# pyannote/pyannote-audio

Measured on AMD Instinct MI355X. Metric: audio-hours/sec (real-time factor) for speaker-diarization-3.1 pipeline, higher is better.
Workload: dtype f32

## Files before the change

include/pyannote_amd.h:

```cpp
#ifndef PYANNOTE_AMD_H
#define PYANNOTE_AMD_H

#include <stddef.h>
#include <stdint.h>

#ifdef __cplusplus
extern "C" {
#endif

int pa_version(void);
const char* pa_last_error(void);

void pa_prof_enable(int on);
size_t pa_prof_report(char* buf, size_t cap);

#define PA_MAX_LSTM_LAYERS 8
#define PA_MAX_LINEAR 4

typedef struct pa_seg_weights {
  int32_t sinc_stride;
  int32_t lstm_layers;
  int32_t lstm_hidden;
  int32_t lstm_bidir;
  int32_t num_linear;
// ... 42 lines not shown
int pa_sinc_fix_pool(const float* S, long Pc, int positions_per_chunk_step, int B, int P, const float* mean,
                     const float* rstd, float gamma, float beta, const float* filt_packed, float* tap_sums,
                     float* out, void* stream);
int pa_sinc_fir_span_centred(const float* wav, long wav_len, long span, const float* mean0, const float* rstd0,
                             const float* filt_packed, float* S, void* stream);
int pa_sinc_fix_pool_centred(const float* S, long Pc, int positions_per_chunk_step, int B, int P, const float* wav,
                             long wav_len, int N, const float* mean, const float* rstd, float gamma, float beta,
                             const float* filt_packed, float* tap_sums, float* out, void* stream);
int pa_conv5_pool(const float* xin, int B, int cin, int Lin, const float* in_mean,
                  const float* in_rstd, const float* gam, const float* bet, const float* w_packed,
                  const float* bias64, float* out, void* stream);
int pa_norm_transpose(const float* xin, int B, int T, const float* in_mean, const float* in_rstd,
                      const float* gam, const float* bet, float* X0, void* stream);
int pa_gemm_tn_ex(const float* A, int lda, const float* W, int ldw, const float* bias, const float* Res,
                  float* C, long ldc, int M, int N, int K, int act, int out_mode, void* stream);
int pa_gemm_tn(const float* A, int lda, const float* W, int ldw, const float* bias, float* C, long ldc,
               int M, int N, int K, int act, int out_mode, void* stream);
int pa_gemm_tn_s2(const float* X, int B, int H, int W, int cin, const float* Wt, int ldw, const float* bias, float* C,
                  long ldc, int N, void* stream);
int pa_lstm_rec(const float* xproj, const float* whh_packed, float* out, int ntiles, int ndir, int T,
                void* stream);
int pa_lstm_rec_h(const float* xproj, const float* whh_packed, float* out, int ntiles, int ndir, int T, int H,
                  void* stream);
int pa_classifier(const float* X, int ldx, int K, int ntiles, int T, int B, const float* cw,
                  const float* cb, int NC, const unsigned char* mapping, int S, float* logp,
                  unsigned char* multilabel, void* stream);

#define PA_MAX_RES_BLOCKS 128

typedef struct pa_emb_weights {
  int32_t num_mel;
  int32_t embed_dim;
  int32_t num_layers;
  int32_t num_blocks[4];
  int32_t planes[4];
  int32_t bottleneck;
  const float* fb_window;
  const float* fb_tw256;
  const float* fb_tw512;
  const float* fb_mel_w;
  const int32_t* fb_mel_lo;
  const int32_t* fb_mel_hi;
  const float* stem_w;
  const float* stem_shift;
  const float* blk_w1[PA_MAX_RES_BLOCKS];
  const float* blk_shift1[PA_MAX_RES_BLOCKS];
  const float* blk_w2[PA_MAX_RES_BLOCKS];
  const float* blk_shift2[PA_MAX_RES_BLOCKS];
  const float* blk_u1[PA_MAX_RES_BLOCKS];
  const float* blk_u2[PA_MAX_RES_BLOCKS];
  const float* blk_wsc[PA_MAX_RES_BLOCKS];
  const float* blk_shiftsc[PA_MAX_RES_BLOCKS];
  const float* blk_w3[PA_MAX_RES_BLOCKS];
  const float* blk_shift3[PA_MAX_RES_BLOCKS];
  const float* seg1_w;
  const float* seg1_b;
  const float* blk_v1[PA_MAX_RES_BLOCKS];
  const float* blk_v2[PA_MAX_RES_BLOCKS];
  int32_t fb_center_kernel;
} pa_emb_weights;

int pa_emb_num_fbank_frames(int num_samples);
int pa_emb_num_pool_frames(const pa_emb_weights* w, int num_samples);
size_t pa_emb_workspace_bytes(const pa_emb_weights* w, int num_chunks, int num_samples, int num_masks);
int pa_emb_forward(const pa_emb_weights* w, const float* wav, int64_t wav_len, int64_t chunk_stride,
                   int num_chunks, int num_samples, const float* masks, int num_masks, int mask_frames,
                   const int32_t* nearest_idx, float* emb, void* workspace, size_t workspace_bytes,
                   void* stream);

size_t pa_emb_ragged_workspace_bytes(const pa_emb_weights* w, int num_utterances, int max_samples);
int pa_emb_forward_ragged(const pa_emb_weights* w, const float* wav, int64_t wav_len, const int64_t* offsets,
                          const int32_t* lengths, int num_utterances, int max_samples, const float* masks, float* emb,
                          void* workspace, size_t workspace_bytes, void* stream);

size_t pa_emb_calibrate_workspace_bytes(const pa_emb_weights* w, int num_chunks, int num_samples);
int pa_emb_calibrate_winograd(const pa_emb_weights* w, const float* wav, int64_t wav_len, int64_t chunk_stride,
                              int num_chunks, int num_samples, float* report, float* emb, void* workspace,
                              size_t workspace_bytes, void* stream);
int pa_absmax_diff(const float* got, const float* ref, long n, float* out2, void* stream);

int pa_fbank(const float* wav, long wav_len, long chunk_stride, int B, int N, const float* window,
             const float* tw256, const float* tw512, const float* mel_w, const int* mel_lo,
             const int* mel_hi, int nmel, float* out, int center, void* stream);
int pa_fbank_center_span(const float* fb, int B, int T, int nmel, int kernel, float* out, void* stream);
int pa_resnet_stem(const float* fbank, int B, int T, int F, const float* w9, const float* shift,
                   float* out, void* stream);
int pa_conv3x3(const float* X, int B, int H, int W, int cin, const float* Wg, const float* shift,
               const float* R, float* Y, int cout, int stride, int relu, void* stream);
int pa_conv3x3_s2_sc_supported(int H, int cin, int cout);
int pa_conv3x3_s2_sc(const float* X, int B, int H, int W, int cin, const float* Wg, const float* shift,
                     const float* Wsc, const float* shift_sc, float* Y, float* Ysc, int cout, int relu,
                     void* stream);
int pa_winograd_pack_host(const float* conv_weight ,
                          const float* bn_scale , int cout, int cin,
                          float* U_slabs );
int pa_conv3x3_wino(const float* X, int B, int H, int W, int cin, const float* U, const float* shift,
                    const float* R, float* Y, int cout, int relu, void* stream);
int pa_winograd4_pack_host(const float* conv_weight ,
                           const float* bn_scale , int cout, int cin,
                           float* U_slabs );
int pa_conv3x3_wino4(const float* X, int B, int H, int W, int cin, const float* U, const float* shift,
                     const float* R, float* Y, int cout, int relu, void* stream);
int pa_conv3x3_wino4_rows(const float* X, int B, int H, int W, int cin, const float* U, const float* shift,
                          const float* R, float* Y, int cout, int relu, int rows, void* stream);
int pa_conv3x3_wino_rows(const float* X, int B, int H, int W, int cin, const float* U, const float* shift,
                         const float* R, float* Y, int cout, int relu, int y_first, void* stream);
int pa_stats_pool(const float* feat, int B, int Fh, int Tp, int C, const float* masks, int S, int Fm,
                  const int* nearest_idx, float* stats, void* stream);
int pa_fbank_ragged(const float* wav, long wav_len, const int64_t* offsets, const int32_t* lengths, int B,
                    int max_samples, const float* window, const float* tw256, const float* tw512, const float* mel_w,
                    const int* mel_lo, const int* mel_hi, int nmel, float* out, void* stream);
int pa_zero_tail_cols(float* x, int B, int H, int W, int C, const int32_t* lengths, int halvings, void* stream);
int pa_stats_pool_ragged(const float* feat, int B, int Fh, int W, int C, const int32_t* lengths, int halvings,
                         const float* masks, int ld_masks, float* stats, void* stream);

#define PA_W2V_MAX_CONV 8
#define PA_W2V_MAX_LAYERS 24
typedef struct pa_w2v_layer {
  const float* qk_w;
  const float* qk_b;
  const float* v_w;
  const float* out_w;
  const float* out_b;
  const float* ln1_g;
  const float* ln1_b;
  const float* ff1_w;
  const float* ff1_b;
  const float* ff2_w;
  const float* ff2_b;
  const float* ln2_g;
  const float* ln2_b;
  const float* gate_w;
  const float* gate_b;
  const float* gate_const;
} pa_w2v_layer;

typedef struct pa_sser_weights {
  int32_t num_conv;
  int32_t conv_channels[PA_W2V_MAX_CONV];
  int32_t conv_kernel[PA_W2V_MAX_CONV];
  int32_t conv_stride[PA_W2V_MAX_CONV];
  int32_t extractor_layer_norm;
  int32_t embed_dim, num_layers, num_heads, ff_dim, layer_norm_first;
  int32_t pos_kernel, pos_groups;
  int32_t wavlm;
  int32_t use_layer;
  int32_t lstm_layers, lstm_hidden, lstm_bidir, num_linear, linear_hidden, num_classes, num_speakers;
  const float* conv_w[PA_W2V_MAX_CONV];
  const float* conv_b[PA_W2V_MAX_CONV];
  const float* conv_norm_g[PA_W2V_MAX_CONV];
  const float* conv_norm_b[PA_W2V_MAX_CONV];
  const float* proj_ln_g;
  const float* proj_ln_b;
  const float* proj_w;
  const float* proj_b;
  const float* pos_w;
  const float* pos_b;
  const float* enc_ln_g;
  const float* enc_ln_b;
  pa_w2v_layer layers[PA_W2V_MAX_LAYERS];
  float layer_mix[PA_W2V_MAX_LAYERS];
  const float* lstm_wih[PA_MAX_LSTM_LAYERS];
  const float* lstm_bias[PA_MAX_LSTM_LAYERS];
  const float* lstm_whh[PA_MAX_LSTM_LAYERS];
  const float* lin_w[PA_MAX_LINEAR];
  const float* lin_b[PA_MAX_LINEAR];
// ... 249 lines not shown
```

pyannote-audio_amd/csrc/emb_fbank.hip:

```cpp
#include "common.h"

namespace pa {

constexpr int FB_WIN = 400, FB_SHIFT = 160, FB_NFFT = 512, FB_HALF = 256, FB_NBIN = 257;
constexpr int FB_FPB = 4;

struct cplx {
  float x, y;
};
__device__ __forceinline__ cplx cmul(cplx a, cplx b) {
  return {a.x * b.x - a.y * b.y, a.x * b.y + a.y * b.x};
}

template <bool kRagged>
__global__ __launch_bounds__(256) void k_fbank(const float* __restrict__ wav, long wav_len,
                                               long chunk_stride, int T, float scale, float preemph,
                                               const float* __restrict__ window,
                                               const float2* __restrict__ tw256,
                                               const float2* __restrict__ tw512,
                                               const float* __restrict__ mel_w,
                                               const int* __restrict__ mel_lo,
                                               const int* __restrict__ mel_hi, int nmel, float eps,
                                               float* __restrict__ out, const int64_t* __restrict__ offs,
                                               const int* __restrict__ lens) {
  __shared__ float2 bufA[FB_FPB][FB_HALF];
  __shared__ float2 bufB[FB_FPB][FB_HALF];
  __shared__ float2 s_tw256[FB_HALF];
  __shared__ float xs[FB_FPB][FB_NFFT + 1];
  const int tid = threadIdx.x, lane = tid & 63, wv = tid >> 6;
  const int b = blockIdx.y;
  const int t = blockIdx.x * FB_FPB + wv;
  int Tb = T;
  long base = (long)b * chunk_stride + (long)t * FB_SHIFT;
  if constexpr (kRagged) {
    const int n = lens[b];
    Tb = n < FB_WIN ? 0 : 1 + (n - FB_WIN) / FB_SHIFT;
    if ((int)blockIdx.x * FB_FPB >= Tb) return;
    base = offs[b] + (long)t * FB_SHIFT;
  }
  for (int i = tid; i < FB_HALF; i += 256) s_tw256[i] = tw256[i];
  const bool active = t < Tb;
  float2 w512[5];
#pragma unroll
  for (int i = 0; i < 5; ++i) w512[i] = lane + 64 * i <= FB_HALF ? tw512[lane + 64 * i] : make_float2(0.f, 0.f);

  float x[7];
  float s = 0.f;
#pragma unroll
  for (int i = 0; i < 7; ++i) {
    const int j = lane + 64 * i;
    float v = 0.f;
    if (active && j < FB_WIN) {
      const long g = base + j;
      v = (g < wav_len ? wav[g] : 0.f) * scale;
    }
    x[i] = v;
    s += v;
  }
  const float mean = wave_sum(s) / (float)FB_WIN;
  float* xw = xs[wv];
#pragma unroll
  for (int i = 0; i < 7; ++i) {
    const int j = lane + 64 * i;
    if (j < FB_WIN) xw[j + 1] = x[i] - mean;
  }
  if (lane == 0) xw[0] = x[0] - mean;
  __syncthreads();
  float y[8];
#pragma unroll
  for (int i = 0; i < 8; ++i) {
    const int j = lane + 64 * i;
    float v = 0.f;
    if (j < FB_WIN) v = (xw[j + 1] - preemph * xw[j]) * window[j];
    y[i] = v;
  }
  __syncthreads();
#pragma unroll
  for (int i = 0; i < 8; ++i) xw[lane + 64 * i] = y[i];
  __syncthreads();
  float2* A = bufA[wv];
  float2* Bf = bufB[wv];
#pragma unroll
  for (int i = 0; i < 4; ++i) {
    const int n = lane + 64 * i;
    A[n] = make_float2(xw[2 * n], xw[2 * n + 1]);
  }
  __syncthreads();

  float2* src = A;
  float2* dst = Bf;
#pragma unroll
  for (int pass = 0; pass < 4; ++pass) {
    const int Ns = 1 << (2 * pass);
    const int j = lane;
    const int k = j & (Ns - 1);
    const int tstep = 64 >> (2 * pass);
    cplx v[4];
#pragma unroll
    for (int r = 0; r < 4; ++r) {
      const float2 d = src[j + 64 * r];
      const float2 w = s_tw256[(r * k * tstep) & 255];
      v[r] = cmul({d.x, d.y}, {w.x, w.y});
    }
    const cplx t0 = {v[0].x + v[2].x, v[0].y + v[2].y};
    const cplx t1 = {v[0].x - v[2].x, v[0].y - v[2].y};
    const cplx t2 = {v[1].x + v[3].x, v[1].y + v[3].y};
    const cplx d13 = {v[1].x - v[3].x, v[1].y - v[3].y};
    const cplx t3 = {d13.y, -d13.x};
    const int j0 = ((j - k) << 2) + k;
    dst[j0] = make_float2(t0.x + t2.x, t0.y + t2.y);
    dst[j0 + Ns] = make_float2(t1.x + t3.x, t1.y + t3.y);
    dst[j0 + 2 * Ns] = make_float2(t0.x - t2.x, t0.y - t2.y);
    dst[j0 + 3 * Ns] = make_float2(t1.x - t3.x, t1.y - t3.y);
    __syncthreads();
    float2* tmp = src;
    src = dst;
    dst = tmp;
  }
#pragma unroll
  for (int i = 0; i < 5; ++i) {
    const int k = lane + 64 * i;
    if (k <= FB_HALF) {
      const float2 zk = src[k & 255];
      const float2 zc0 = src[(FB_HALF - k) & 255];
      const cplx zc = {zc0.x, -zc0.y};
      const cplx e = {0.5f * (zk.x + zc.x), 0.5f * (zk.y + zc.y)};
      const cplx dd = {0.5f * (zk.x - zc.x), 0.5f * (zk.y - zc.y)};
      const cplx o = {dd.y, -dd.x};
      const float2 w = w512[i];
      const cplx wo = cmul(o, {w.x, w.y});
      const float re = e.x + wo.x, im = e.y + wo.y;
      xw[k] = re * re + im * im;
    }
  }
  __syncthreads();
  if (active) {
    for (int m = lane; m < nmel; m += 64) {
      const float* wrow = mel_w + (long)m * FB_NBIN;
      float acc = 0.f;
      const int lo = mel_lo[m], hi = mel_hi[m];
      for (int k0 = lo; k0 <= hi; k0 += 8) {
        float wk[8];
#pragma unroll
        for (int u = 0; u < 8; ++u) wk[u] = k0 + u <= hi ? wrow[k0 + u] : 0.f;
#pragma unroll
        for (int u = 0; u < 8; ++u)
          if (k0 + u <= hi) acc = fmaf(xw[k0 + u], wk[u], acc);
      }
      out[((long)b * T + t) * nmel + m] = logf(fmaxf(acc, eps));
    }
  }
}

__global__ __launch_bounds__(320) void k_fbank_center(float* __restrict__ fb, int T, int nmel) {
  __shared__ float part[4][80];
  const int b = blockIdx.x;
  const int m = threadIdx.x % 80, p = threadIdx.x / 80;
  float* x = fb + (long)b * T * nmel;
  float s = 0.f;
  if (m < nmel)
    for (int t = p; t < T; t += 4) s += x[(long)t * nmel + m];
  part[p][m] = s;
  __syncthreads();
  const float mean = (part[0][m] + part[1][m] + part[2][m] + part[3][m]) / (float)T;
  if (m < nmel)
    for (int t = p; t < T; t += 4) x[(long)t * nmel + m] -= mean;
}

__global__ __launch_bounds__(320) void k_fbank_center_ragged(float* __restrict__ fb, int T, int nmel,
                                                             const int* __restrict__ lens) {
  __shared__ float part[4][80];
  const int b = blockIdx.x;
  const int m = threadIdx.x % 80, p = threadIdx.x / 80;
  const int n = lens[b];
  const int Tb = n < FB_WIN ? 0 : 1 + (n - FB_WIN) / FB_SHIFT;
  float* x = fb + (long)b * T * nmel;
  float s = 0.f;
  if (m < nmel)
    for (int t = p; t < Tb; t += 4) s += x[(long)t * nmel + m];
  part[p][m] = s;
  __syncthreads();
  const float mean = (part[0][m] + part[1][m] + part[2][m] + part[3][m]) / (float)Tb;
  if (m < nmel) {
    for (int t = p; t < Tb; t += 4) x[(long)t * nmel + m] -= mean;
    for (int t = Tb + p; t < T; t += 4) x[(long)t * nmel + m] = 0.f;
  }
}

constexpr int FC_TT = 240, FC_MG = 16, FC_KMAX = 2049;
__global__ __launch_bounds__(256) void k_fbank_center_span(const float* __restrict__ fb, int T, int nmel, int K,
                                                           float* __restrict__ out) {
  extern __shared__ float fc_tile[];
  const int b = blockIdx.z, m0 = blockIdx.y * FC_MG, t0 = blockIdx.x * FC_TT;
  const int half = K >> 1;
  const int m = threadIdx.x & (FC_MG - 1), tl = threadIdx.x >> 4;
  const float* x = fb + (long)b * T * nmel;
  const int rows = FC_TT + K - 1;
  for (int r = tl; r < rows; r += 16) {
    const int t = t0 - half + r;
    fc_tile[r * FC_MG + m] = (t >= 0 && t < T && m0 + m < nmel) ? x[(long)t * nmel + m0 + m] : 0.f;
  }
  __syncthreads();
  if (m0 + m >= nmel) return;
  for (int i = tl; i < FC_TT; i += 16) {
    const int t = t0 + i;
    if (t >= T) break;
    const int lo = t - half < 0 ? 0 : t - half, hi = t + half > T - 1 ? T - 1 : t + half;
    float s = 0.f;
    for (int u = lo; u <= hi; ++u) s += fc_tile[(u - t0 + half) * FC_MG + m];
    out[((long)b * T + t) * nmel + m0 + m] = fc_tile[(i + half) * FC_MG + m] - s / (float)(hi - lo + 1);
  }
}

}

extern "C" {

int pa_fbank_center_span(const float* fb, int B, int T, int nmel, int kernel, float* out, void* stream) {
  PA_REQUIRE(kernel >= 1 && (kernel & 1), "pa_fbank_center_span: the window must be an odd number of frames (got %d)",
             kernel);
  PA_REQUIRE(fb != out, "pa_fbank_center_span: works out of place");
  if (B <= 0 || T <= 0 || nmel <= 0) return 0;
  if (kernel > 2 * T - 1) kernel = 2 * T - 1;
  PA_REQUIRE(kernel <= pa::FC_KMAX,
             "pa_fbank_center_span: a running mean over %d frames of a %d-frame chunk needs more than the LDS holds "
             "(at most %d frames)", kernel, T, pa::FC_KMAX);
  const size_t lds = (size_t)(pa::FC_TT + kernel - 1) * pa::FC_MG * sizeof(float);
  static bool attr_set = false;
  if (!attr_set) {
    (void)hipFuncSetAttribute((const void*)pa::k_fbank_center_span, hipFuncAttributeMaxDynamicSharedMemorySize,
                              (int)((pa::FC_TT + pa::FC_KMAX - 1) * pa::FC_MG * sizeof(float)));
    attr_set = true;
  }
  hipLaunchKernelGGL(pa::k_fbank_center_span, dim3(pa::cdiv(T, pa::FC_TT), pa::cdiv(nmel, pa::FC_MG), B), dim3(256), lds,
                     (hipStream_t)stream, fb, T, nmel, kernel, out);
  PA_CHECK_LAUNCH("pa_fbank_center_span");
  return 0;
}

int pa_fbank(const float* wav, long wav_len, long chunk_stride, int B, int N, const float* window,
             const float* tw256, const float* tw512, const float* mel_w, const int* mel_lo,
             const int* mel_hi, int nmel, float* out, int center, void* stream) {
  PA_REQUIRE(nmel <= 80, "pa_fbank: at most 80 mel bins are built (got %d)", nmel);
  if (B <= 0) return 0;
  PA_REQUIRE(N >= pa::FB_WIN, "pa_fbank: %d samples is shorter than one 25 ms frame", N);
  const int T = 1 + (N - pa::FB_WIN) / pa::FB_SHIFT;
  hipStream_t st = (hipStream_t)stream;
  pa::ProfScope prof("k_fbank", stream, (double)B * T * (5.0 * 512 * 9 + 2.0 * 257 * 3 + 2.0 * 257 * 2),
                     4.0 * B * N + 4.0 * B * T * nmel * (center ? 3 : 1));
  hipLaunchKernelGGL(pa::k_fbank<false>, dim3(pa::cdiv(T, pa::FB_FPB), B), dim3(256), 0, st, wav, wav_len,
                     chunk_stride, T, 32768.0f, 0.97f, window, (const float2*)tw256,
                     (const float2*)tw512, mel_w, mel_lo, mel_hi, nmel, 1.1920928955078125e-07f, out,
                     (const int64_t*)nullptr, (const int*)nullptr);
  PA_CHECK_LAUNCH("pa_fbank");
  if (center) {
    hipLaunchKernelGGL(pa::k_fbank_center, dim3(B), dim3(320), 0, st, out, T, nmel);
    PA_CHECK_LAUNCH("pa_fbank_center");
  }
  return 0;
}

int pa_fbank_ragged(const float* wav, long wav_len, const int64_t* offsets, const int32_t* lengths, int B,
                    int max_samples, const float* window, const float* tw256, const float* tw512, const float* mel_w,
                    const int* mel_lo, const int* mel_hi, int nmel, float* out, void* stream) {
  PA_REQUIRE(nmel <= 80, "pa_fbank_ragged: at most 80 mel bins are built (got %d)", nmel);
  if (B <= 0) return 0;
  PA_REQUIRE(max_samples >= pa::FB_WIN, "pa_fbank_ragged: %d samples is shorter than one 25 ms frame", max_samples);
  const int T = 1 + (max_samples - pa::FB_WIN) / pa::FB_SHIFT;
  hipStream_t st = (hipStream_t)stream;
  pa::ProfScope prof("k_fbank_ragged", stream, (double)B * T * (5.0 * 512 * 9 + 2.0 * 257 * 3 + 2.0 * 257 * 2),
                     4.0 * B * max_samples + 12.0 * B * T * nmel);
  hipLaunchKernelGGL(pa::k_fbank<true>, dim3(pa::cdiv(T, pa::FB_FPB), B), dim3(256), 0, st, wav, wav_len, 0L, T,
                     32768.0f, 0.97f, window, (const float2*)tw256, (const float2*)tw512, mel_w, mel_lo, mel_hi, nmel,
                     1.1920928955078125e-07f, out, offsets, (const int*)lengths);
  PA_CHECK_LAUNCH("pa_fbank_ragged");
  hipLaunchKernelGGL(pa::k_fbank_center_ragged, dim3(B), dim3(320), 0, st, out, T, nmel, (const int*)lengths);
  PA_CHECK_LAUNCH("pa_fbank_center_ragged");
  return 0;
}

}
```

pyannote-audio_amd/csrc/emb_forward.cpp:

```cpp
#include "forward_common.h"

namespace {

struct EmbPlan {
  int B, N, T, F, S;
  int Hs[5], Ws[5];
  size_t fbank, act[4], stats, total, act_elems;
  size_t t2_off, gather_off;
};

inline bool s2_fold_wanted() {
  static const bool fold = getenv("PA_S2_FOLD") == nullptr || atoi(getenv("PA_S2_FOLD")) != 0;
  return fold;
}

inline bool prefer_wino4(int H, int W, int cin) {
  auto up = [](int a, int b) { return (long)((a + b - 1) / b) * b; };
  long p4 = up(H, 4) * up(W, 64);
  const long p4_lin = up(H, 4) * up(W, 4);
  if (p4_lin * 120 <= p4 * 100) p4 = p4_lin * 120 / 100;
  long p2 = up(H, 8) * up(W, 32);
  if (up(H, 4) * up(W, 64) < p2) p2 = up(H, 4) * up(W, 64);
  if (up(H, 2) * up(W, 128) < p2) p2 = up(H, 2) * up(W, 128);
  const long gain = cin >= 256 ? 130 : 122;
  return p4 * 100 <= p2 * gain;
}

bool make_plan(const pa_emb_weights* w, int B, int N, int S, EmbPlan* p, bool calib = false) {
  if (N < 400) return false;
  p->B = B;
  p->N = N;
  p->S = S < 1 ? 1 : S;
  p->T = 1 + (N - 400) / 160;
  p->F = w->num_mel;
  p->Hs[0] = p->F;
  p->Ws[0] = p->T;
  for (int l = 0; l < w->num_layers; ++l) {
    const int s = l == 0 ? 1 : 2;
    p->Hs[l + 1] = (p->Hs[l] - 1) / s + 1;
    p->Ws[l + 1] = (p->Ws[l] - 1) / s + 1;
  }
  pa::Bump ws;
  p->fbank = ws.take((size_t)B * p->T * p->F);
  const int ex = w->bottleneck ? 4 : 1;
  p->act_elems = (size_t)B * p->Hs[0] * p->Ws[0] * w->planes[0] * ex;
  for (int i = 0; i < 3; ++i) p->act[i] = ws.take(p->act_elems);
  p->t2_off = p->gather_off = 0;
  if (w->bottleneck) {
    size_t t1 = 0, t2 = 0, g = 0;
    int cin = w->planes[0];
    for (int l = 0; l < w->num_layers; ++l) {
      const size_t planes = w->planes[l];
      const size_t in_px = (size_t)B * p->Hs[l == 0 ? 1 : l] * p->Ws[l == 0 ? 1 : l];
      const size_t out_px = (size_t)B * p->Hs[l + 1] * p->Ws[l + 1];
      t1 = t1 > in_px * planes ? t1 : in_px * planes;
      t2 = t2 > out_px * planes ? t2 : out_px * planes;
      if (l > 0) g = g > out_px * cin ? g : out_px * cin;
      cin = 4 * (int)planes;
    }
    p->t2_off = pa::Bump::align(t1);
    p->gather_off = p->t2_off + pa::Bump::align(t2);
    p->act[3] = ws.take(p->gather_off + pa::Bump::align(g));
  } else if (calib) {
    p->act[3] = ws.take(p->act_elems);
  }
  const int L = w->num_layers;
  p->stats = ws.take((size_t)B * p->S * 2 * w->planes[L - 1] * ex * p->Hs[L]);
  p->total = ws.o;
  return true;
}

}

extern "C" {

int pa_emb_num_fbank_frames(int num_samples) {
  return num_samples < 400 ? 0 : 1 + (num_samples - 400) / 160;
}

int pa_emb_num_pool_frames(const pa_emb_weights* w, int num_samples) {
  EmbPlan p;
  if (!make_plan(w, 1, num_samples, 1, &p)) return 0;
  return p.Ws[w->num_layers];
}

size_t pa_emb_workspace_bytes(const pa_emb_weights* w, int num_chunks, int num_samples, int num_masks) {
  EmbPlan p;
  if (!make_plan(w, num_chunks, num_samples, num_masks, &p)) return 0;
  return p.total * sizeof(float);
}

}


static int emb_forward_impl(const pa_emb_weights* w, const float* wav, int64_t wav_len, int64_t chunk_stride,
                            int num_chunks, int num_samples, const float* masks, int num_masks, int mask_frames,
                            const int32_t* nearest_idx, float* emb, void* workspace, size_t workspace_bytes,
                            void* stream, float* calib, const int64_t* offsets = nullptr,
                            const int32_t* lengths = nullptr) {
  if (num_chunks <= 0) return 0;
  const bool ragged = lengths != nullptr;
  EmbPlan p;
  if (w->num_layers != 4 || !make_plan(w, num_chunks, num_samples, masks ? num_masks : 1, &p, calib != nullptr)) {
    pa::set_error("pa_emb_forward: %d samples is too short (fbank needs >= 400) or bad layer count",
                  num_samples);
    return 3;
  }
  if (workspace_bytes < p.total * sizeof(float)) {
    pa::set_error("pa_emb_forward: workspace too small (%zu < %zu bytes)", workspace_bytes,
                  p.total * sizeof(float));
    return 3;
  }
  float* ws = (float*)workspace;
  const int B = p.B;

  const int span = w->fb_center_kernel;
  if (ragged && span != 0) {
    pa::set_error("pa_emb_forward_ragged: fbank_centering_span checkpoints run one launch sequence per length");
    return 3;
  }
  if (ragged)
    PA_RUN(pa_fbank_ragged(wav, wav_len, offsets, lengths, B, p.N, w->fb_window, w->fb_tw256, w->fb_tw512, w->fb_mel_w,
                           w->fb_mel_lo, w->fb_mel_hi, w->num_mel, ws + p.fbank, stream));
  else
    PA_RUN(pa_fbank(wav, wav_len, chunk_stride, B, p.N, w->fb_window, w->fb_tw256, w->fb_tw512, w->fb_mel_w,
                    w->fb_mel_lo, w->fb_mel_hi, w->num_mel, ws + p.fbank, span == 0 ? 1 : 0, stream));
  auto zero_tail = [&](float* X, int l, int C) -> int {
    return ragged ? pa_zero_tail_cols(X, B, p.Hs[l], p.Ws[l], C, lengths, l > 0 ? l - 1 : 0, stream) : 0;
  };
  float* cur = ws + p.act[0];
  float* f1 = ws + p.act[1];
  float* f2 = ws + p.act[2];
  const float* feats = ws + p.fbank;
  if (span != 0) {
    PA_RUN(pa_fbank_center_span(ws + p.fbank, B, p.T, p.F, span, f1, stream));
    feats = f1;
  }
  PA_RUN(pa_resnet_stem(feats, B, p.T, p.F, w->stem_w, w->stem_shift, cur, stream));
  if (!w->bottleneck) PA_RUN(zero_tail(cur, 0, w->planes[0]));

  auto conv_s1 = [&](const float* X, int H, int W, int ci, const float* v, const float* u, const float* wd,
                     const float* shift, const float* R, float* Y, int co, int slot) -> int {
    if (calib != nullptr) {
      float* scratch = ws + p.act[3];
      float* rep = calib + 4 * slot;
      const long n = (long)B * H * W * co;
      int r = pa_conv3x3(X, B, H, W, ci, wd, shift, R, Y, co, 1, 1, stream);
      if (r == 0 && v != nullptr) {
        r = pa_conv3x3_wino4(X, B, H, W, ci, v, shift, R, scratch, co, 1, stream);
        if (r == 0) r = pa_absmax_diff(scratch, Y, n, rep, stream);
      }
      if (r == 0 && u != nullptr) {
        r = pa_conv3x3_wino(X, B, H, W, ci, u, shift, R, scratch, co, 1, stream);
        if (r == 0) r = pa_absmax_diff(scratch, Y, n, rep + 2, stream);
      }
      return r;
    }
    if (v != nullptr && prefer_wino4(H, W, ci)) return pa_conv3x3_wino4(X, B, H, W, ci, v, shift, R, Y, co, 1, stream);
    if (u != nullptr) return pa_conv3x3_wino(X, B, H, W, ci, u, shift, R, Y, co, 1, stream);
    return pa_conv3x3(X, B, H, W, ci, wd, shift, R, Y, co, 1, 1, stream);
  };

  int blk = 0;
  int cin = w->planes[0];
  if (w->bottleneck) {
    float* nxt = f1;
    float* sc = f2;
    float* tmp = ws + p.act[3];
    for (int l = 0; l < w->num_layers; ++l) {
      const int planes = w->planes[l], cout = 4 * planes;
      for (int i = 0; i < w->num_blocks[l]; ++i, ++blk) {
        if (blk >= PA_MAX_RES_BLOCKS) {
          pa::set_error("pa_emb_forward: more than %d residual blocks", PA_MAX_RES_BLOCKS);
          return 3;
        }
        const int stride = (i == 0 && l > 0) ? 2 : 1;
        const int H = stride == 2 ? p.Hs[l] : p.Hs[l + 1], W = stride == 2 ? p.Ws[l] : p.Ws[l + 1];
        const int Ho = p.Hs[l + 1], Wo = p.Ws[l + 1];
        float* t1 = tmp;
        float* t2 = tmp + p.t2_off;
        PA_RUN(pa_gemm_tn_ex(cur, cin, w->blk_w1[blk], cin, w->blk_shift1[blk], nullptr, t1, planes, B * H * W,
                             planes, cin, 2, 0, stream));
        PA_RUN(zero_tail(t1, stride == 2 ? l : l + 1, planes));
        if (stride == 1 && w->blk_u2[blk] != nullptr)
          PA_RUN(pa_conv3x3_wino(t1, B, H, W, planes, w->blk_u2[blk], w->blk_shift2[blk], nullptr, t2, planes, 1,
                                 stream));
        else
          PA_RUN(pa_conv3x3(t1, B, H, W, planes, w->blk_w2[blk], w->blk_shift2[blk], nullptr, t2, planes, stride,
                            1, stream));
        const float* res = cur;
        if (w->blk_wsc[blk] != nullptr) {
          if (stride == 2)
            PA_RUN(pa_gemm_tn_s2(cur, B, H, W, cin, w->blk_wsc[blk], cin, w->blk_shiftsc[blk], sc, cout, cout, stream));
          else
            PA_RUN(pa_gemm_tn_ex(cur, cin, w->blk_wsc[blk], cin, w->blk_shiftsc[blk], nullptr, sc, cout,
                                 B * Ho * Wo, cout, cin, 0, 0, stream));
          res = sc;
        } else if (stride != 1 || cin != cout) {
          pa::set_error("pa_emb_forward: block %d needs a shortcut conv but none was given", blk);
          return 3;
        }
        PA_RUN(pa_gemm_tn_ex(t2, planes, w->blk_w3[blk], planes, w->blk_shift3[blk], res, nxt, cout, B * Ho * Wo,
                             cout, planes, 2, 0, stream));
        float* t = cur;
        cur = nxt;
        nxt = t;
// ... 112 lines not shown
```

pyannote-audio_amd/ffi.py:

```python
from __future__ import annotations

import ctypes as C
from pathlib import Path

import torch

_LIB = None
PA_MAX_LSTM_LAYERS = 8
PA_MAX_LINEAR = 4

c_fp = C.c_void_p


class SegWeights(C.Structure):
    _fields_ = [
        ("sinc_stride", C.c_int32), ("lstm_layers", C.c_int32), ("lstm_hidden", C.c_int32),
        ("lstm_bidir", C.c_int32), ("num_linear", C.c_int32), ("linear_hidden", C.c_int32),
        ("num_classes", C.c_int32), ("num_speakers", C.c_int32),
        ("wav_gamma", C.c_float), ("wav_beta", C.c_float),
        ("sinc_filt", c_fp), ("norm0", c_fp), ("conv1_w", c_fp), ("conv1_b", c_fp), ("norm1", c_fp),
        ("conv2_w", c_fp), ("conv2_b", c_fp), ("norm2", c_fp),
        ("lstm_wih", c_fp * PA_MAX_LSTM_LAYERS), ("lstm_bias", c_fp * PA_MAX_LSTM_LAYERS),
        ("lstm_whh", c_fp * PA_MAX_LSTM_LAYERS),
        ("lin_w", c_fp * PA_MAX_LINEAR), ("lin_b", c_fp * PA_MAX_LINEAR),
# ... 91 lines not shown
class LibraryNotBuilt(RuntimeError):
    pass


def lib_path() -> Path:
    import os
    if os.environ.get("PA_LIB"):
        return Path(os.environ["PA_LIB"])
    return Path(__file__).resolve().parent / "libpyannote_amd.so"


def load():
    global _LIB
    if _LIB is not None:
        return _LIB
    p = lib_path()
    if not p.exists():
        raise LibraryNotBuilt(
            f"{p} not found: run `python -c 'import __graft_entry__ as g; g.build()'` "
            "(hipcc --offload-arch=gfx950).  There is no CPU fallback.")
    lib = C.CDLL(str(p))
    lib.pa_last_error.restype = C.c_char_p
    lib.pa_version.restype = C.c_int
    lib.pa_seg_workspace_bytes.restype = C.c_size_t
    lib.pa_seg_workspace_bytes.argtypes = [C.POINTER(SegWeights), C.c_int, C.c_int]
    lib.pa_seg_workspace_bytes_strided.restype = C.c_size_t
    lib.pa_seg_workspace_bytes_strided.argtypes = [C.POINTER(SegWeights), C.c_int, C.c_int, C.c_int64]
    lib.pa_seg_num_frames.argtypes = [C.c_int, C.c_int]
    lib.pa_seg_forward.argtypes = [C.POINTER(SegWeights), c_fp, C.c_int64, C.c_int64, C.c_int, C.c_int,
                                   c_fp, c_fp, c_fp, C.c_size_t, c_fp]
    lib.pa_row_stats.argtypes = [c_fp, C.c_long, C.c_long, C.c_int, C.c_int, C.c_float, c_fp, c_fp, c_fp]
    lib.pa_sinc_fir_pool.argtypes = [c_fp, C.c_long, C.c_long, C.c_int, C.c_int, C.c_int, c_fp, c_fp,
                                     C.c_float, C.c_float, c_fp, c_fp, c_fp]
    lib.pa_sinc_fir_span.argtypes = [c_fp, C.c_long, C.c_long, c_fp, c_fp, c_fp]
    lib.pa_sinc_fix_pool.argtypes = [c_fp, C.c_long, C.c_int, C.c_int, C.c_int, c_fp, c_fp, C.c_float, C.c_float,
                                     c_fp, c_fp, c_fp, c_fp]
    lib.pa_sinc_fir_span_centred.argtypes = [c_fp, C.c_long, C.c_long, c_fp, c_fp, c_fp, c_fp, c_fp]
    lib.pa_sinc_fix_pool_centred.argtypes = [c_fp, C.c_long, C.c_int, C.c_int, C.c_int, c_fp, C.c_long, C.c_int, c_fp,
                                             c_fp, C.c_float, C.c_float, c_fp, c_fp, c_fp, c_fp]
    lib.pa_conv5_pool.argtypes = [c_fp, C.c_int, C.c_int, C.c_int, c_fp, c_fp, c_fp, c_fp, c_fp, c_fp,
                                  c_fp, c_fp]
    lib.pa_norm_transpose.argtypes = [c_fp, C.c_int, C.c_int, c_fp, c_fp, c_fp, c_fp, c_fp, c_fp]
    lib.pa_gemm_tn_ex.argtypes = [c_fp, C.c_int, c_fp, C.c_int, c_fp, c_fp, c_fp, C.c_long, C.c_int, C.c_int,
                                  C.c_int, C.c_int, C.c_int, c_fp]
    lib.pa_gemm_tn.argtypes = [c_fp, C.c_int, c_fp, C.c_int, c_fp, c_fp, C.c_long, C.c_int, C.c_int,
                               C.c_int, C.c_int, C.c_int, c_fp]
    lib.pa_lstm_rec.argtypes = [c_fp, c_fp, c_fp, C.c_int, C.c_int, C.c_int, c_fp]
    lib.pa_classifier.argtypes = [c_fp, C.c_int, C.c_int, C.c_int, C.c_int, C.c_int, c_fp, c_fp,
                                  C.c_int, c_fp, C.c_int, c_fp, c_fp, c_fp]
    lib.pa_prof_enable.argtypes = [C.c_int]
    lib.pa_prof_enable.restype = None
    lib.pa_prof_report.argtypes = [C.c_char_p, C.c_size_t]
    lib.pa_prof_report.restype = C.c_size_t
    _declare_optional(lib)
    _LIB = lib
    return lib


_OPTIONAL: list[tuple] = [
    ("pa_emb_num_fbank_frames", [C.c_int], C.c_int),
    ("pa_emb_num_pool_frames", [C.POINTER(EmbWeights), C.c_int], C.c_int),
    ("pa_emb_workspace_bytes", [C.POINTER(EmbWeights), C.c_int, C.c_int, C.c_int], C.c_size_t),
    ("pa_emb_forward", [C.POINTER(EmbWeights), c_fp, C.c_int64, C.c_int64, C.c_int, C.c_int, c_fp,
                        C.c_int, C.c_int, c_fp, c_fp, c_fp, C.c_size_t, c_fp], C.c_int),
    ("pa_emb_ragged_workspace_bytes", [C.POINTER(EmbWeights), C.c_int, C.c_int], C.c_size_t),
    ("pa_emb_forward_ragged", [C.POINTER(EmbWeights), c_fp, C.c_int64, c_fp, c_fp, C.c_int, C.c_int, c_fp, c_fp,
                               c_fp, C.c_size_t, c_fp], C.c_int),
    ("pa_fbank_ragged", [c_fp, C.c_long, c_fp, c_fp, C.c_int, C.c_int, c_fp, c_fp, c_fp, c_fp, c_fp, c_fp, C.c_int,
                         c_fp, c_fp], C.c_int),
    ("pa_zero_tail_cols", [c_fp, C.c_int, C.c_int, C.c_int, C.c_int, c_fp, C.c_int, c_fp], C.c_int),
    ("pa_stats_pool_ragged", [c_fp, C.c_int, C.c_int, C.c_int, C.c_int, c_fp, C.c_int, c_fp, C.c_int, c_fp, c_fp],
     C.c_int),
    ("pa_emb_calibrate_workspace_bytes", [C.POINTER(EmbWeights), C.c_int, C.c_int], C.c_size_t),
    ("pa_emb_calibrate_winograd", [C.POINTER(EmbWeights), c_fp, C.c_int64, C.c_int64, C.c_int, C.c_int, c_fp, c_fp,
                                   c_fp, C.c_size_t, c_fp], C.c_int),
    ("pa_lstm_rec_h", [c_fp, c_fp, c_fp, C.c_int, C.c_int, C.c_int, C.c_int, c_fp], C.c_int),
    ("pa_absmax_diff", [c_fp, c_fp, C.c_long, c_fp, c_fp], C.c_int),
    ("pa_gemm_tn_s2", [c_fp, C.c_int, C.c_int, C.c_int, C.c_int, c_fp, C.c_int, c_fp, c_fp, C.c_long, C.c_int,
                       c_fp], C.c_int),
    ("pa_gemm_tn_batched", [c_fp, C.c_int, C.c_long, C.c_long, c_fp, C.c_int, C.c_long, C.c_long, c_fp, c_fp, C.c_long,
                            C.c_long, C.c_long, C.c_int, C.c_int, C.c_int, C.c_int, C.c_int, C.c_int, c_fp], C.c_int),
    ("pa_fbank", [c_fp, C.c_long, C.c_long, C.c_int, C.c_int, c_fp, c_fp, c_fp, c_fp, c_fp, c_fp,
                  C.c_int, c_fp, C.c_int, c_fp], C.c_int),
    ("pa_fbank_center_span", [c_fp, C.c_int, C.c_int, C.c_int, C.c_int, c_fp, c_fp], C.c_int),
    ("pa_resnet_stem", [c_fp, C.c_int, C.c_int, C.c_int, c_fp, c_fp, c_fp, c_fp], C.c_int),
    ("pa_conv3x3", [c_fp, C.c_int, C.c_int, C.c_int, C.c_int, c_fp, c_fp, c_fp, c_fp, C.c_int, C.c_int,
                    C.c_int, c_fp], C.c_int),
    ("pa_conv3x3_s2_sc_supported", [C.c_int, C.c_int, C.c_int], C.c_int),
    ("pa_conv3x3_s2_sc", [c_fp, C.c_int, C.c_int, C.c_int, C.c_int, c_fp, c_fp, c_fp, c_fp, c_fp, c_fp, C.c_int,
                          C.c_int, c_fp], C.c_int),
    ("pa_conv3x3_wino", [c_fp, C.c_int, C.c_int, C.c_int, C.c_int, c_fp, c_fp, c_fp, c_fp, C.c_int, C.c_int,
                         c_fp], C.c_int),
    ("pa_conv3x3_wino4", [c_fp, C.c_int, C.c_int, C.c_int, C.c_int, c_fp, c_fp, c_fp, c_fp, C.c_int, C.c_int,
                          c_fp], C.c_int),
    ("pa_conv3x3_wino4_rows", [c_fp, C.c_int, C.c_int, C.c_int, C.c_int, c_fp, c_fp, c_fp, c_fp, C.c_int, C.c_int,
                               C.c_int, c_fp], C.c_int),
    ("pa_conv3x3_wino_rows", [c_fp, C.c_int, C.c_int, C.c_int, C.c_int, c_fp, c_fp, c_fp, c_fp, C.c_int, C.c_int,
                              C.c_int, c_fp], C.c_int),
    ("pa_pdist_f64", [c_fp, C.c_int, C.c_int, c_fp, c_fp], C.c_int),
    ("pa_cdist_cosine_f64", [c_fp, C.c_int, c_fp, C.c_int, C.c_int, c_fp, c_fp, c_fp], C.c_int),
    ("pa_centroid_means", [c_fp, C.c_int, c_fp, c_fp, C.c_int, c_fp, c_fp], C.c_int),
    ("pa_linkage_workspace_bytes", [C.c_int], C.c_size_t),
    ("pa_linkage_centroid_f64", [c_fp, C.c_int, c_fp, c_fp, C.c_size_t, c_fp], C.c_int),
    ("pa_pdist_cosine_f64", [c_fp, C.c_int, C.c_int, c_fp, c_fp, c_fp], C.c_int),
    ("pa_nonfinite_flag_f64", [c_fp, C.c_long, c_fp, c_fp], C.c_int),
    ("pa_linkage_chain_workspace_bytes", [C.c_int], C.c_size_t),
    ("pa_linkage_chain_f64", [c_fp, C.c_int, C.c_int, c_fp, c_fp, C.c_size_t, c_fp], C.c_int),
    ("pa_seg_files_workspace_bytes", [C.POINTER(SegWeights), C.c_int, c_fp, C.c_int, C.c_int64], C.c_size_t),
    ("pa_seg_forward_files", [C.POINTER(SegWeights), c_fp, c_fp, c_fp, C.c_int, C.c_int64, C.c_int, c_fp, c_fp, c_fp,
                              C.c_size_t, c_fp], C.c_int),
    ("pa_gather_chunks", [c_fp, c_fp, c_fp, c_fp, C.c_int, C.c_int, c_fp, c_fp], C.c_int),
    ("pa_seg_chunk_stats", [c_fp, C.c_int, C.c_int, C.c_int, c_fp, c_fp, c_fp], C.c_int),
    ("pa_embedding_masks", [c_fp, C.c_int, C.c_int, C.c_int, c_fp, C.c_int, C.c_int, c_fp, c_fp], C.c_int),
    ("pa_speaker_count", [c_fp, C.c_int, C.c_int, C.c_int, c_fp, C.c_int, c_fp, c_fp, c_fp], C.c_int),
    ("pa_cluster_activations", [c_fp, C.c_int, C.c_int, C.c_int, c_fp, c_fp, C.c_int, C.c_int, c_fp, c_fp],
     C.c_int),
    ("pa_topk_binarize", [c_fp, c_fp, C.c_int, C.c_int, C.c_int, c_fp, c_fp, c_fp], C.c_int),
    ("pa_topk_binarize_f32", [c_fp, c_fp, C.c_int, C.c_int, C.c_int, c_fp, c_fp, c_fp], C.c_int),
    ("pa_binarize_hysteresis", [c_fp, C.c_int, C.c_int, C.c_int, C.c_float, C.c_float, C.c_float, C.c_int, c_fp,
                                c_fp], C.c_int),
    ("pa_cluster_max", [c_fp, C.c_int, C.c_int, C.c_int, c_fp, C.c_int, c_fp, c_fp], C.c_int),
    ("pa_aggregate", [c_fp, C.c_int, C.c_int, C.c_int, c_fp, C.c_int, c_fp, c_fp, C.c_float, C.c_float, C.c_int,
                      c_fp, c_fp], C.c_int),
    ("pa_binarize_regions_workspace_bytes", [C.c_int, C.c_int, C.c_int], C.c_size_t),
    ("pa_binarize_regions", [c_fp, C.c_int, C.c_int, c_fp, c_fp, c_fp, c_fp, C.c_double, C.c_double, C.c_double,
                             C.c_int, c_fp, c_fp, c_fp, c_fp, C.c_size_t, c_fp], C.c_int),
    ("pa_regions_sweep_groups", [C.c_int, C.c_int, c_fp], C.c_int),
    ("pa_regions_sweep_workspace_bytes", [C.c_int, C.c_int, C.c_int, C.c_int, C.c_int, C.c_long, C.c_long],
     C.c_size_t),
    ("pa_regions_sweep_count", [c_fp, C.c_int, C.c_int, C.c_int, c_fp, c_fp, c_fp, c_fp, c_fp, c_fp, C.c_size_t,
                                c_fp], C.c_int),
    ("pa_regions_sweep_emit", [c_fp, C.c_int, C.c_int, C.c_int, c_fp, c_fp, c_fp, c_fp, C.c_int, c_fp, c_fp, c_fp,
                               C.c_double, C.c_double, C.c_double, C.c_long, c_fp, c_fp, c_fp, c_fp, c_fp, C.c_size_t,
                               c_fp], C.c_int),
    ("pa_resample_poly", [c_fp, C.c_long, c_fp, C.c_int, C.c_int, C.c_int, C.c_int, c_fp, C.c_long, c_fp],
     C.c_int),
    ("pa_plda_transform", [c_fp, C.c_int, C.c_int, C.c_int, C.c_int, c_fp, c_fp, c_fp, c_fp, c_fp, c_fp, c_fp],
     C.c_int),
    ("pa_vbx_workspace_bytes", [C.c_int, C.c_int, C.c_int], C.c_size_t),
    ("pa_vbx_iteration", [c_fp, c_fp, C.c_int, C.c_int, C.c_int, C.c_double, C.c_double, C.c_int, c_fp, c_fp,
                          c_fp, C.c_size_t, c_fp], C.c_int),
    ("pa_vbx_batch_workspace_bytes", [C.c_int, C.c_int, C.c_int, C.c_int], C.c_size_t),
    ("pa_vbx_run_batch", [c_fp, c_fp, C.c_int, C.c_int, C.c_int, c_fp, C.c_long, c_fp, c_fp, C.c_int, C.c_int,
                          C.c_double, c_fp, c_fp, c_fp, c_fp, C.c_size_t, c_fp], C.c_int),
    ("pa_constrained_assign_max_speakers", [], C.c_int),
    ("pa_constrained_assign_max_clusters", [], C.c_int),
    ("pa_constrained_assign", [c_fp, c_fp, C.c_int, C.c_int, C.c_int, c_fp, c_fp, c_fp], C.c_int),
    ("pa_stats_pool", [c_fp, C.c_int, C.c_int, C.c_int, C.c_int, c_fp, C.c_int, C.c_int, c_fp, c_fp,
                       c_fp], C.c_int),
    ("pa_stats_pool_rows", [c_fp, C.c_int, C.c_int, C.c_int, C.c_int, C.c_int, c_fp, C.c_int, C.c_int, c_fp,
                            c_fp, C.c_int, c_fp, c_fp, c_fp], C.c_int),
    ("pa_sser_num_frames", [C.POINTER(SserWeights), C.c_int], C.c_int),
    ("pa_sser_workspace_bytes", [C.POINTER(SserWeights), C.c_int, C.c_int], C.c_size_t),
    ("pa_sser_forward", [C.POINTER(SserWeights), c_fp, C.c_int64, C.c_int64, C.c_int, C.c_int, c_fp, c_fp, c_fp,
                         c_fp, C.c_size_t, c_fp], C.c_int),
    ("pa_w2v_conv0", [c_fp, C.c_long, C.c_long, C.c_int, C.c_int, C.c_int, C.c_int, C.c_int, C.c_int, C.c_int, c_fp,
                      c_fp, c_fp, c_fp], C.c_int),
    ("pa_w2v_group_norm_gelu", [c_fp, C.c_int, C.c_int, C.c_int, C.c_int, c_fp, c_fp, c_fp, c_fp, c_fp], C.c_int),
    ("pa_w2v_layernorm", [c_fp, c_fp, C.c_long, C.c_int, c_fp, c_fp, C.c_int, c_fp], C.c_int),
    ("pa_w2v_posconv", [c_fp, C.c_int, C.c_int, C.c_int, C.c_int, C.c_int, C.c_int, c_fp, c_fp, c_fp, c_fp], C.c_int),
    ("pa_w2v_softmax", [c_fp, C.c_int, C.c_int, C.c_int, C.c_int, C.c_float, c_fp, c_fp, C.c_int, C.c_int, c_fp, c_fp,
                        c_fp, c_fp], C.c_int),
    ("pa_w2v_axpy", [c_fp, c_fp, C.c_float, C.c_long, C.c_int, c_fp], C.c_int),
    ("pa_w2v_to_tiles", [c_fp, C.c_int, C.c_int, C.c_int, C.c_int, c_fp, c_fp], C.c_int),
    ("pa_xvec_num_frames", [C.POINTER(XvecWeights), C.c_int], C.c_int),
    ("pa_xvec_workspace_bytes", [C.POINTER(XvecWeights), C.c_int, C.c_int, C.c_int], C.c_size_t),
# ... 105 lines not shown
```

Baseline: 1.328.

## Compute fbank frames once across overlapping sliding-window chunks

When embedding chunks are uniform sliding windows whose stride is a multiple of the 160-sample frame shift, the log-mel frames of the whole overlapping span are computed once into a scratch buffer. A new centering kernel then gathers each chunk's frames, subtracts the per-chunk mean and writes the usual fbank layout. This avoids recomputing the FFT and mel filterbank for frames shared by overlapping chunks. It reuses an activation workspace slot as scratch and depends on chunk start alignment; it is on by default and can be disabled with an environment variable.

```diff
diff --git a/include/pyannote_amd.h b/include/pyannote_amd.h
--- a/include/pyannote_amd.h
+++ b/include/pyannote_amd.h
@@ -148,6 +148,9 @@
 int pa_fbank(const float* wav, long wav_len, long chunk_stride, int B, int N, const float* window,
              const float* tw256, const float* tw512, const float* mel_w, const int* mel_lo,
              const int* mel_hi, int nmel, float* out, int center, void* stream);
+int pa_fbank_shared(const float* wav, long wav_len, long chunk_stride, int B, int N, const float* window,
+                    const float* tw256, const float* tw512, const float* mel_w, const int* mel_lo,
+                    const int* mel_hi, int nmel, float* frames, float* out, void* stream);
 int pa_fbank_center_span(const float* fb, int B, int T, int nmel, int kernel, float* out, void* stream);
 int pa_resnet_stem(const float* fbank, int B, int T, int F, const float* w9, const float* shift,
                    float* out, void* stream);
diff --git a/pyannote-audio_amd/csrc/emb_fbank.hip b/pyannote-audio_amd/csrc/emb_fbank.hip
--- a/pyannote-audio_amd/csrc/emb_fbank.hip
+++ b/pyannote-audio_amd/csrc/emb_fbank.hip
@@ -1,8 +1,9 @@
 #include "common.h"
+#include "emb_fbank_shared.h"
 
 namespace pa {
 
-constexpr int FB_WIN = 400, FB_SHIFT = 160, FB_NFFT = 512, FB_HALF = 256, FB_NBIN = 257;
+constexpr int FB_NFFT = 512, FB_HALF = 256, FB_NBIN = 257;
 constexpr int FB_FPB = 4;
 
 struct cplx {
@@ -152,19 +153,36 @@
   }
 }
 
+__device__ __forceinline__ float fbank_chunk_mean(const float* __restrict__ x, int T, int nmel, int m, int p,
+                                                  float (*part)[80]) {
+  float s = 0.f;
+  if (m < nmel)
+    for (int t = p; t < T; t += 4) s += x[(long)t * nmel + m];
+  part[p][m] = s;
+  __syncthreads();
+  return (part[0][m] + part[1][m] + part[2][m] + part[3][m]) / (float)T;
+}
+
 __global__ __launch_bounds__(320) void k_fbank_center(float* __restrict__ fb, int T, int nmel) {
   __shared__ float part[4][80];
   const int b = blockIdx.x;
   const int m = threadIdx.x % 80, p = threadIdx.x / 80;
   float* x = fb + (long)b * T * nmel;
-  float s = 0.f;
-  if (m < nmel)
-    for (int t = p; t < T; t += 4) s += x[(long)t * nmel + m];
-  part[p][m] = s;
-  __syncthreads();
-  const float mean = (part[0][m] + part[1][m] + part[2][m] + part[3][m]) / (float)T;
+  const float mean = fbank_chunk_mean(x, T, nmel, m, p, part);
   if (m < nmel)
     for (int t = p; t < T; t += 4) x[(long)t * nmel + m] -= mean;
+}
+
+__global__ __launch_bounds__(320) void k_fbank_center_shared(const float* __restrict__ frames, int hop, int T, int nmel,
+                                                             float* __restrict__ out) {
+  __shared__ float part[4][80];
+  const int b = blockIdx.x;
+  const int m = threadIdx.x % 80, p = threadIdx.x / 80;
+  const float* x = frames + (long)b * hop * nmel;
+  float* y = out + (long)b * T * nmel;
+  const float mean = fbank_chunk_mean(x, T, nmel, m, p, part);
+  if (m < nmel)
+    for (int t = p; t < T; t += 4) y[(long)t * nmel + m] = x[(long)t * nmel + m] - mean;
 }
 
 __global__ __launch_bounds__(320) void k_fbank_center_ragged(float* __restrict__ fb, int T, int nmel,
@@ -260,6 +278,30 @@
   return 0;
 }
 
+int pa_fbank_shared(const float* wav, long wav_len, long chunk_stride, int B, int N, const float* window,
+                    const float* tw256, const float* tw512, const float* mel_w, const int* mel_lo,
+                    const int* mel_hi, int nmel, float* frames, float* out, void* stream) {
+  PA_REQUIRE(nmel <= 80, "pa_fbank_shared: at most 80 mel bins are built (got %d)", nmel);
+  pa::FbankShared s;
+  PA_REQUIRE(pa::fbank_shared_plan(chunk_stride, B, N, &s),
+             "pa_fbank_shared: %d chunks of %d samples, %ld apart, do not share frames (needs two or more chunks, a "
+             "stride of 160 k > 0 samples and fewer frames between chunks than in one)", B, N, chunk_stride);
+  hipStream_t st = (hipStream_t)stream;
+  const int Tf = (int)s.Tf;
+  {
+    pa::ProfScope prof("k_fbank_shared", stream, (double)Tf * (5.0 * 512 * 9 + 2.0 * 257 * 3 + 2.0 * 257 * 2),
+                       4.0 * ((double)Tf * pa::FB_SHIFT + pa::FB_WIN - pa::FB_SHIFT) + 4.0 * Tf * nmel);
+    hipLaunchKernelGGL(pa::k_fbank<false>, dim3(pa::cdiv(Tf, pa::FB_FPB), 1), dim3(256), 0, st, wav, wav_len, 0L, Tf,
+                       32768.0f, 0.97f, window, (const float2*)tw256, (const float2*)tw512, mel_w, mel_lo, mel_hi, nmel,
+                       1.1920928955078125e-07f, frames, (const int64_t*)nullptr, (const int*)nullptr);
+    PA_CHECK_LAUNCH("pa_fbank_shared");
+  }
+  pa::ProfScope prof("k_fbank_center_shared", stream, 2.0 * B * s.T * nmel, 4.0 * Tf * nmel + 4.0 * B * s.T * nmel);
+  hipLaunchKernelGGL(pa::k_fbank_center_shared, dim3(B), dim3(320), 0, st, (const float*)frames, s.hop, s.T, nmel, out);
+  PA_CHECK_LAUNCH("pa_fbank_center_shared");
+  return 0;
+}
+
 int pa_fbank_ragged(const float* wav, long wav_len, const int64_t* offsets, const int32_t* lengths, int B,
                     int max_samples, const float* window, const float* tw256, const float* tw512, const float* mel_w,
                     const int* mel_lo, const int* mel_hi, int nmel, float* out, void* stream) {
diff --git a/pyannote-audio_amd/csrc/emb_fbank_shared.h b/pyannote-audio_amd/csrc/emb_fbank_shared.h
--- /dev/null
+++ b/pyannote-audio_amd/csrc/emb_fbank_shared.h
@@ -0,0 +1,28 @@
+#pragma once
+#include <stdint.h>
+
+namespace pa {
+
+constexpr int FB_WIN = 400, FB_SHIFT = 160;
+constexpr int64_t FBS_MAX_FRAMES = (int64_t)1 << 30;
+
+struct FbankShared {
+  int T;
+  int hop;
+  int64_t Tf;
+};
+
+inline bool fbank_shared_plan(int64_t chunk_stride, int B, int N, FbankShared* s) {
+  if (B < 2 || N < FB_WIN || chunk_stride <= 0 || chunk_stride % FB_SHIFT != 0) return false;
+  const int T = 1 + (N - FB_WIN) / FB_SHIFT;
+  const int64_t hop = chunk_stride / FB_SHIFT;
+  if (hop >= T) return false;
+  const int64_t Tf = (int64_t)(B - 1) * hop + T;
+  if (Tf > FBS_MAX_FRAMES) return false;
+  s->T = T;
+  s->hop = (int)hop;
+  s->Tf = Tf;
+  return true;
+}
+
+}
diff --git a/pyannote-audio_amd/csrc/emb_forward.cpp b/pyannote-audio_amd/csrc/emb_forward.cpp
--- a/pyannote-audio_amd/csrc/emb_forward.cpp
+++ b/pyannote-audio_amd/csrc/emb_forward.cpp
@@ -1,3 +1,4 @@
+#include "emb_fbank_shared.h"
 #include "forward_common.h"
 
 namespace {
@@ -12,6 +13,11 @@
 inline bool s2_fold_wanted() {
   static const bool fold = getenv("PA_S2_FOLD") == nullptr || atoi(getenv("PA_S2_FOLD")) != 0;
   return fold;
+}
+
+inline bool shared_fbank_wanted() {
+  static const bool shared = getenv("PA_EMB_SHARED_FBANK") == nullptr || atoi(getenv("PA_EMB_SHARED_FBANK")) != 0;
+  return shared;
 }
 
 inline bool prefer_wino4(int H, int W, int cin) {
@@ -119,9 +125,15 @@
     pa::set_error("pa_emb_forward_ragged: fbank_centering_span checkpoints run one launch sequence per length");
     return 3;
   }
+  pa::FbankShared fs;
+  const bool shared = !ragged && span == 0 && calib == nullptr && shared_fbank_wanted() &&
+                      pa::fbank_shared_plan(chunk_stride, B, p.N, &fs);
   if (ragged)
     PA_RUN(pa_fbank_ragged(wav, wav_len, offsets, lengths, B, p.N, w->fb_window, w->fb_tw256, w->fb_tw512, w->fb_mel_w,
                            w->fb_mel_lo, w->fb_mel_hi, w->num_mel, ws + p.fbank, stream));
+  else if (shared)
+    PA_RUN(pa_fbank_shared(wav, wav_len, chunk_stride, B, p.N, w->fb_window, w->fb_tw256, w->fb_tw512, w->fb_mel_w,
+                           w->fb_mel_lo, w->fb_mel_hi, w->num_mel, ws + p.act[1], ws + p.fbank, stream));
   else
     PA_RUN(pa_fbank(wav, wav_len, chunk_stride, B, p.N, w->fb_window, w->fb_tw256, w->fb_tw512, w->fb_mel_w,
                     w->fb_mel_lo, w->fb_mel_hi, w->num_mel, ws + p.fbank, span == 0 ? 1 : 0, stream));
diff --git a/pyannote-audio_amd/ffi.py b/pyannote-audio_amd/ffi.py
--- a/pyannote-audio_amd/ffi.py
+++ b/pyannote-audio_amd/ffi.py
@@ -197,6 +197,8 @@
                             C.c_long, C.c_long, C.c_int, C.c_int, C.c_int, C.c_int, C.c_int, C.c_int, c_fp], C.c_int),
     ("pa_fbank", [c_fp, C.c_long, C.c_long, C.c_int, C.c_int, c_fp, c_fp, c_fp, c_fp, c_fp, c_fp,
                   C.c_int, c_fp, C.c_int, c_fp], C.c_int),
+    ("pa_fbank_shared", [c_fp, C.c_long, C.c_long, C.c_int, C.c_int, c_fp, c_fp, c_fp, c_fp, c_fp, c_fp,
+                         C.c_int, c_fp, c_fp, c_fp], C.c_int),
     ("pa_fbank_center_span", [c_fp, C.c_int, C.c_int, C.c_int, C.c_int, c_fp, c_fp], C.c_int),
     ("pa_resnet_stem", [c_fp, C.c_int, C.c_int, C.c_int, c_fp, c_fp, c_fp, c_fp], C.c_int),
     ("pa_conv3x3", [c_fp, C.c_int, C.c_int, C.c_int, C.c_int, c_fp, c_fp, c_fp, c_fp, C.c_int, C.c_int,
```

After: 1.338 (median of 6 runs). No clear change (+0.8%).
